# AlterPang/Multi_ORB_SLAM

Hardware: AMD Instinct MI355X
Metric: frames/sec (N-cam extract+match) (higher is better)
Workload: dtype u8; 1 GPU; configs[1]: one 2-cam 640x480 rig per GPU, 8-level pyramid, 1000 feat/cam; HIP FAST+rBRIEF extract + SearchByProjection + cross-camera Hamming top-2; cams_per_gpu=2, rig_cams=2, rigs=1, width=640, height=480, nfeatures=1000, nlevels=8, frame_unit=one rig timestep (2 cameras)

## Files before the change

multi_orb_slam_amd/csrc/resolve_dev.h:

```cpp
#pragma once
#include <hip/hip_runtime.h>
#include <cstddef>
#include <type_traits>
#include "../../include/orbm.h"
#include "orb_common.h"
#include "matcher_internal.h"

namespace morb {

static __host__ __device__ __forceinline__ int rotation_bin(float query_angle, float feature_angle) {
    float rot = query_angle - feature_angle;
    if (rot < 0.0) rot += 360.0f;
    int bin = (int)roundf(rot * (1.0f / ORBM_HISTO_LENGTH));
    if (bin == ORBM_HISTO_LENGTH) bin = 0;
    return (bin >= 0 && bin < ORBM_HISTO_LENGTH) ? bin : -1;
}

static __host__ __device__ __forceinline__ void three_maxima(const int* histo, int L, int* ind) {
    int m1 = 0, m2 = 0, m3 = 0, i1 = -1, i2 = -1, i3 = -1;
    for (int i = 0; i < L; i++) {
        const int s = histo[i];
        if (s > m1) { m3 = m2; i3 = i2; m2 = m1; i2 = i1; m1 = s; i1 = i; }
        else if (s > m2) { m3 = m2; i3 = i2; m2 = s; i2 = i; }
        else if (s > m3) { m3 = s; i3 = i; }
// ... 6 lines not shown
static __device__ __forceinline__ void three_maxima_wave(int sv, int lane, int keep[3]) {
    int rank = 0;
#pragma unroll
    for (int j = 0; j < ORBM_HISTO_LENGTH; ++j) {
        const int sj = __builtin_amdgcn_readlane(sv, j);
        rank += (sj > sv || (sj == sv && j < lane)) ? 1 : 0;
    }
    const bool in = lane < ORBM_HISTO_LENGTH && sv > 0;
    const unsigned long long r1 = __ballot(in && rank == 0), r2 = __ballot(in && rank == 1), r3 = __ballot(in && rank == 2);
    int i1 = r1 ? __ffsll((long long)r1) - 1 : -1, i2 = r2 ? __ffsll((long long)r2) - 1 : -1, i3 = r3 ? __ffsll((long long)r3) - 1 : -1;
    const int m1 = i1 >= 0 ? __builtin_amdgcn_readlane(sv, i1) : 0, m2 = i2 >= 0 ? __builtin_amdgcn_readlane(sv, i2) : 0,
              m3 = i3 >= 0 ? __builtin_amdgcn_readlane(sv, i3) : 0;
    if ((float)m2 < 0.1f * (float)m1) { i2 = -1; i3 = -1; }
    else if ((float)m3 < 0.1f * (float)m1) { i3 = -1; }
    keep[0] = i1; keep[1] = i2; keep[2] = i3;
}

static __device__ __forceinline__ void hist_add_wave(int* s_hist, bool in_range, int bin, int lane) {
    unsigned long long todo = __ballot(in_range);
    for (int rounds = 0; todo && rounds < 3; ++rounds) {
        const int b0 = __builtin_amdgcn_readlane(bin, __ffsll((long long)todo) - 1);
        const unsigned long long same = __ballot(in_range && bin == b0);
        if (in_range && bin == b0 && lane == __ffsll((long long)same) - 1) atomicAdd(&s_hist[b0], __popcll(same));
        todo &= ~same;
    }
    if (in_range && ((todo >> lane) & 1)) atomicAdd(&s_hist[bin], 1);
}

struct Rescan { int k1, g1, k2; };
template <bool SECOND, typename Hidden>
static __device__ __forceinline__ Rescan rescan_wave(int q, int full, int nq, const int* __restrict__ cand_idx,
                                                     const uint16_t* __restrict__ cand_dist, const uint8_t* __restrict__ occupied,
                                                     int lane, Hidden hidden) {
    int k1 = 0x7fffffff, k2 = 0x7fffffff, g1 = -1;
    for (int k0 = 0; k0 < full; k0 += 64) {
        const int k = k0 + lane;
        int key = 0x7fffffff, g = -1;
        if (k < full) {
            g = cand_idx[k * nq + q];
            const int d = cand_dist[k * nq + q];
            bool avail = !(occupied && occupied[g]);
            if (hidden(g, q)) avail = false;
            if (avail) key = (d << 16) | k;
        }
        const int m1 = (int)wave_min_u32((unsigned)key);
        int m2 = 0x7fffffff;
        if (SECOND) m2 = (int)wave_min_u32((unsigned)(key == m1 ? 0x7fffffff : key));
        if (m1 < k1) {
            k2 = min(k1, m2); k1 = m1;
            g1 = __builtin_amdgcn_readlane(g, __ffsll((long long)__ballot(key == m1)) - 1);
        }
        else k2 = min(k2, m1);
    }
    return {k1, g1, k2};
}

struct Advance { int nk, ne; };
template <int K>
static __device__ __forceinline__ void shortlist_claims(const int (&e)[K], int p, bool displaced, const int* claims, int (&ck)[K]) {
#pragma unroll
    for (int k = 1; k < K; ++k) {
        const bool want = displaced && k > p && e[k] != 0xffff;
        const int v = claims[want ? e[k] : 0];
        ck[k] = want ? v : -1;
    }
}
template <int K>
static __device__ __forceinline__ Advance shortlist_first_free(const int (&e)[K], const int (&ck)[K], int i) {
    int nk = K;
#pragma unroll
    for (int k = K - 1; k >= 1; --k) if (ck[k] >= i) nk = k;
    int ne = 0xffff;
#pragma unroll
    for (int k = 1; k < K; ++k) if (nk == k) ne = e[k];
    return {nk, ne};
}
template <int K>
static __device__ __forceinline__ Advance shortlist_advance(const int (&e)[K], int p, int i, const int* claims) {
    int ck[K];
    shortlist_claims(e, p, true, claims, ck);
    return shortlist_first_free(e, ck, i);
}

struct RescanCtx {
    int nq; const int* cand_idx; const uint16_t* cand_dist; const uint8_t* occupied; int th_high, f0;
};

template <int RQ, typename Choice, typename Len>
static __device__ inline bool mono_pass(int* claims, const int (&qi)[RQ], const int (&e)[RQ][RESOLVE_K], int (&c)[RQ], int (&p)[RQ],
                                                 const int (&fl)[RQ], Choice l_choice, const RescanCtx& R, Len list_len, int lane,
                                                 unsigned long long* chg) {
    constexpr int K = RESOLVE_K;
    constexpr bool MIRROR = !std::is_same<Choice, std::nullptr_t>::value;
    bool disp[RQ], need_rescan[RQ];
    int cl[RQ];
#pragma unroll
    for (int b = 0; b < RQ; ++b) cl[b] = claims[c[b] >= 0 ? c[b] : 0];
#pragma unroll
    for (int b = 0; b < RQ; ++b) { disp[b] = c[b] >= 0 && cl[b] < qi[b]; need_rescan[b] = false; }
    bool any = false;
#pragma unroll
    for (int b = 0; b < RQ; ++b) any |= disp[b];
    if (!__ballot(any)) return false;
    {
        int ck[RQ][K];
#pragma unroll
        for (int b = 0; b < RQ; ++b) {
            if (!__ballot(disp[b])) continue;
            shortlist_claims(e[b], p[b], disp[b], claims, ck[b]);
        }
#pragma unroll
        for (int b = 0; b < RQ; ++b) {
            if (!__ballot(disp[b])) continue;
            if (!disp[b]) continue;
            const int i = qi[b];
#ifdef MORB_PHASE_CLOCKS
            if (chg) atomicAdd(chg, 1ull);
#endif
            const Advance a = shortlist_first_free(e[b], ck[b], i);
            if (a.nk < K) {
                c[b] = a.ne; p[b] = a.nk;
                if constexpr (MIRROR) l_choice[i] = (unsigned short)a.ne;
                if (fl[b] & 1) atomicMin(&claims[a.ne], i);
            } else {
                c[b] = -1; p[b] = K;
                if constexpr (MIRROR) l_choice[i] = 0xffff;
                need_rescan[b] = (fl[b] & 2) != 0;
            }
        }
    }
#pragma unroll
    for (int b = 0; b < RQ; ++b) {
        unsigned long long todo = __ballot(need_rescan[b]);
#ifdef MORB_PHASE_CLOCKS
        if (todo && lane == 0 && chg) atomicAdd(chg + 16, (unsigned long long)__popcll(todo));
#endif
        while (todo) {
            const int src = __ffsll((long long)todo) - 1;
            todo &= todo - 1;
            const int q = __builtin_amdgcn_readlane(qi[b], src);
            const Rescan r = rescan_wave<false>(q, list_len(q), R.nq, R.cand_idx, R.cand_dist, R.occupied, lane,
                                                [&](int g, int q_) { return claims[g - R.f0] < q_; });
            if (lane == src && r.k1 != 0x7fffffff && (r.k1 >> 16) <= R.th_high) {
                const int g1 = r.g1 - R.f0;
                c[b] = g1;
                if constexpr (MIRROR) l_choice[q] = (unsigned short)g1;
                if (fl[b] & 1) atomicMin(&claims[g1], q);
            }
        }
    }
    return true;
}

static __device__ __forceinline__ void write_matches(int* __restrict__ words, const int* owner, int count, int tagb, int tid, int T) {
    for (int g = tid; g < count; g += T) words[g] = tagb ? (tagb | (owner[g] + 2)) : owner[g];
}
static __device__ __forceinline__ void write_no_match_tail(int* __restrict__ match_of_feature, int NT, int capacity, int tagb, int tid, int T) {
    if (tagb) for (int g = NT + tid; g < capacity; g += T) match_of_feature[g] = tagb | 1;
}

template <typename T>
static __device__ __forceinline__ T* lds_at(int* base, size_t byte_offset) {
    return reinterpret_cast<T*>(reinterpret_cast<unsigned char*>(base) + byte_offset);
}

struct JacobiLds {
    size_t n, nq;
    __host__ __device__ JacobiLds(int n_, int nq_) : n((size_t)n_), nq((size_t)nq_) {}
    __host__ __device__ size_t claim2() const { return 4 * n; }
    __host__ __device__ size_t cnt() const { return 8 * n; }
    __host__ __device__ size_t tables_bytes() const { return cnt() + (nq + 1) / 2 * 4; }
    __host__ __device__ size_t choice() const { return tables_bytes(); }
    __host__ __device__ size_t gd() const { return choice() + 4 * nq; }
    __host__ __device__ size_t ang() const { return gd() + 4 * RESOLVE_K * nq; }
    __host__ __device__ size_t fang() const { return ang() + 4 * nq; }
    __host__ __device__ size_t fl() const { return fang() + 4 * n; }
    __host__ __device__ size_t bytes(bool ldsq) const { return ldsq ? fl() + nq + 16 : tables_bytes(); }
};

struct MonoLds {
    size_t n, nq, nq2;
    bool with_ang;
    __host__ __device__ MonoLds(int n_, int nq_, bool ang_) : n((size_t)n_), nq((size_t)nq_), nq2(((size_t)nq_ + 1) & ~(size_t)1), with_ang(ang_) {}
    __host__ __device__ size_t owner() const { return 4 * n; }
    __host__ __device__ size_t cnt() const { return 8 * n; }
    __host__ __device__ size_t choice() const { return cnt() + 2 * nq2; }
    __host__ __device__ size_t gd() const { return choice() + 2 * nq2; }
    __host__ __device__ size_t fl() const { return gd() + 2 * RESOLVE_K * nq2; }
    __host__ __device__ size_t ang() const { return fl() + ((nq + 3) & ~(size_t)3); }
    __host__ __device__ size_t fang() const { return ang() + 4 * nq; }
    __host__ __device__ size_t wl() const { return with_ang ? fang() + 4 * n : ang(); }
    __host__ __device__ size_t bytes() const { return wl() + 2 * nq2 + 16; }
};

struct CamsLds {
    size_t nf_cap, q_cap;
    __host__ __device__ CamsLds(int nf_cap_, int q_cap_) : nf_cap((size_t)nf_cap_), q_cap((size_t)q_cap_) {}
    __host__ __device__ size_t owner() const { return 4 * nf_cap; }
    __host__ __device__ size_t queries() const { return 8 * nf_cap; }
    __host__ __device__ size_t bytes() const { return queries() + 2 * q_cap; }
};

}
```

multi_orb_slam_amd/csrc/search.hip:

```cpp
#include <algorithm>
#include <cmath>
#include <cstdlib>
#include <type_traits>
#include <vector>

#include "../../include/orbm.h"
#include "../../include/orb_debug.h"
#include "orb_common.h"
#include "frame_sink.h"
#include "matcher_internal.h"
#include "hamming_dev.h"
#include "project_dev.h"
#include "resolve_dev.h"

using namespace morb;

namespace {
__global__ __launch_bounds__(256) void k_project(ProjectArgs A) {
    MORB_LATENCY_KERNEL_WIDE();
    const int qi = __builtin_amdgcn_readfirstlane(blockIdx.x * 4 + (threadIdx.x >> 6));
    if (qi >= A.nq) return;
    project_wave(A, qi, threadIdx.x & 63);
}

// ... 189 lines not shown
                        else {
                            if (found == 0) { best = dk[k]; bidx = gk[k]; }
                            else { best2 = dk[k]; g2 = gk[k]; }
                            if (++found >= NEED) walking = false;
                        }
                    }
                };
#pragma unroll
                for (int k = 0; k < K0; ++k) fetch(k);
#pragma unroll
                for (int k = 0; k < K0; ++k) ck[k] = gk[k] >= 0 ? rd[gk[k]] : 0x7fffffff;
#pragma unroll
                for (int k = 0; k < K0; ++k) walk(k);
                if (__ballot(walking)) {
#pragma unroll
                    for (int k = K0; k < RESOLVE_K; ++k) fetch(k);
#pragma unroll
                    for (int k = K0; k < RESOLVE_K; ++k) ck[k] = gk[k] >= 0 ? rd[gk[k]] : 0x7fffffff;
#pragma unroll
                    for (int k = K0; k < RESOLVE_K; ++k) walk(k);
                }
                if (POINTS) { if (bidx >= 0) lvl = F.octave[bidx]; if (g2 >= 0) lvl2 = F.octave[g2]; }
                need_rescan = found < NEED && (fl & 2) && taken > 0;
                if (!need_rescan && best <= th_high && bidx >= 0) {
                    nc = bidx;
                    if (POINTS && lvl == lvl2 && (float)best > nnratio * (float)best2) nc = -1;
                }
            }
            unsigned long long todo = __ballot(need_rescan);
#ifdef MORB_PHASE_CLOCKS
            if (todo && lane == 0 && it < 15) atomicAdd(&s_nres, __popcll(todo));
#endif
            while (todo) {
                const int src = __ffsll((long long)todo) - 1;
                todo &= todo - 1;
                const int qi = __builtin_amdgcn_readlane(i, src);
                const Rescan r = rescan_wave<POINTS>(qi, l_cnt[qi], nq, cand_idx, cand_dist, occupied, lane,
                                                     [&](int g, int q) { return (unsigned)(rd[g] - tag) < (unsigned)q; });
                int best = 256, best2 = 256, lvl = -1, lvl2 = -1, bidx = -1;
                if (r.k1 != 0x7fffffff) {
                    best = r.k1 >> 16; bidx = r.g1;
                    if (POINTS) lvl = F.octave[bidx];
                }
                if (POINTS && r.k2 != 0x7fffffff) { best2 = r.k2 >> 16; lvl2 = F.octave[cand_idx[(r.k2 & 0xffff) * nq + qi]]; }
                int rnc = -1;
                if (best <= th_high && bidx >= 0) {
                    rnc = bidx;
                    if (POINTS && lvl == lvl2 && (float)best > nnratio * (float)best2) rnc = -1;
                }
                if (lane == src) nc = rnc;
            }
            if (valid) {
#ifdef MORB_PHASE_CLOCKS
                if (nc != old && it < 15) atomicAdd((unsigned long long*)&g_ph_chg[it], 1ull);
#endif
                if (nc != old) { ch = 1; if (LDSQ) l_choice[i] = nc; else choice[i] = nc; }
                if constexpr (B < RQ) chr[B] = nc;
                if (nc >= 0 && (fl & 1)) atomicMin(&wr[nc], tag_next | i);
            }
        };
        batch(0, std::integral_constant<int, 0>{});
        if (T < nq) batch(T, std::integral_constant<int, 1>{});
        if constexpr (RQ > 2) {
            if (2 * T < nq) batch(2 * T, std::integral_constant<int, 2>{});
            if (3 * T < nq) batch(3 * T, std::integral_constant<int, 3>{});
        }
        for (int base = RQ * T; base < nq; base += T) batch(base, std::integral_constant<int, RQ>{});
#ifdef MORB_PHASE_CLOCKS
        __syncthreads();
        if (tid == 0 && it < 15) g_ph_res[40 + it] = (unsigned long long)s_nres;
#endif
        if (it == 0) MORB_PHASE(g_ph_res, 20); else if (it == 5) MORB_PHASE(g_ph_res, 24);
        if (it == 0) MORB_PHASE(g_ph_res, 22); else if (it == 5) MORB_PHASE(g_ph_res, 26);
        changed = __syncthreads_or(ch);
        MORB_PHASE(g_ph_res, min(3 + it, 50));
    }
    if (changed) {
        if (tid == 0) { status[1] = tagb | 0; status[2] = tagb | it; status[3] = tagb | maxcount; status[0] = tagb | 1; }
        return;
    }
    for (int g = tid; g < NT; g += T) s_claim[g] = -1;
    if (tid < ORBM_HISTO_LENGTH) s_hist[tid] = 0;
    if (tid == 0) s_red = 0;
    __syncthreads();
    MORB_PHASE(g_ph_res, 52);
    auto bin_of = [&](int i, int c) { return LDSQ ? rotation_bin(l_ang[i], l_fang[c]) : rotation_bin(__int_as_float(qmeta[i].y), f_angle[c]); };
    int acc = 0;
    for (int i = tid; i < nq; i += T) {
        const int c = LDSQ ? l_choice[i] : choice[i];
        if (c < 0) continue;
        ++acc;
        atomicMax(&s_claim[c], i);
        if (!POINTS && check_ori) {
            const int bin = bin_of(i, c);
            if (LDSQ) l_fl[i] = (unsigned char)((l_fl[i] & 3) | ((bin + 1) << 2));
            hist_add_wave(s_hist, bin >= 0, bin, lane);
        }
    }
    acc = __builtin_amdgcn_readlane(wave_incl_scan(acc), 63);
    if (lane == 0) atomicAdd(&s_red, acc);
    __syncthreads();
    MORB_PHASE(g_ph_res, 53);
    if (!POINTS && check_ori) {
        if (tid < 64) {
            int keep[3];
            three_maxima_wave(tid < ORBM_HISTO_LENGTH ? s_hist[tid] : 0, lane, keep);
            if (tid == 0) { s_keep[0] = keep[0]; s_keep[1] = keep[1]; s_keep[2] = keep[2]; }
        }
        __syncthreads();
        MORB_PHASE(g_ph_res, 54);
        int rej = 0;
        for (int i = tid; i < nq; i += T) {
            const int c = LDSQ ? l_choice[i] : choice[i];
            if (c < 0) continue;
            const int bin = LDSQ ? (int)(l_fl[i] >> 2) - 1 : bin_of(i, c);
            if (bin >= 0 && bin != s_keep[0] && bin != s_keep[1] && bin != s_keep[2]) {
                s_claim[c] = -2;
                ++rej;
            }
        }
        rej = __builtin_amdgcn_readlane(wave_incl_scan(rej), 63);
        if (lane == 0) atomicSub(&s_red, rej);
        __syncthreads();
    }
    MORB_PHASE(g_ph_res, 60);
    write_matches(match_of_feature, s_claim, NT, tagb, tid, T);
    write_no_match_tail(match_of_feature, NT, F.n_total, tagb, tid, T);
    if (tid == 0) { status[1] = tagb | s_red; status[2] = tagb | it; status[3] = tagb | maxcount; status[0] = tagb | 0; }
    MORB_PHASE(g_ph_res, 61);
#ifdef MORB_PHASE_CLOCKS
    if (tid == 0) g_ph_res[62] = (unsigned long long)it;
#endif
}

template <int RQ, bool ANG>
__global__ __launch_bounds__(1024) void k_resolve_mono(FrameDev F, const int2* __restrict__ qmeta, int nq, int cap,
                                                       const int* __restrict__ cand_idx, const uint16_t* __restrict__ cand_dist,
                                                       const int* __restrict__ cand_count, const uint8_t* __restrict__ occupied,
                                                       const float* __restrict__ f_angle, int th_high, int check_ori, int max_it,
                                                       const int* __restrict__ topk, int* __restrict__ match_of_feature,
                                                       int* __restrict__ status, int tagb, MergeJob MJ, int worklist) {
    MORB_LATENCY_KERNEL();
    if (blockIdx.x > 0) { merge_carrier_block(MJ, 1); return; }
    extern __shared__ __attribute__((aligned(16))) int s_claim[];
    __shared__ int s_hist[ORBM_HISTO_LENGTH];
    __shared__ int s_merge_ok;
    __shared__ int s_keep[3];
    __shared__ int s_red;
    __shared__ int s_flag[3];
    const int tid = threadIdx.x, T = blockDim.x;
    const int lane = tid & 63;
    MORB_PHASE(g_ph_res, 0);
#ifdef MORB_PHASE_CLOCKS
    if (tid == 0) { g_ph_res[1] = 0; g_ph_res[58] = clock64(); }
#endif
    if (tid < 3) s_flag[tid] = 0;
    const int NT = F.n_total_dev ? *F.n_total_dev : F.n_total;
    const int* tk_g = topk + RESOLVE_K * nq;
    const MonoLds L(F.n_total, nq, ANG);
    const int nq2 = (int)L.nq2;
    int* s_owner = lds_at<int>(s_claim, L.owner());
    unsigned short* l_cnt = lds_at<unsigned short>(s_claim, L.cnt());
    unsigned short* l_choice = lds_at<unsigned short>(s_claim, L.choice());
    unsigned short* l_gd = lds_at<unsigned short>(s_claim, L.gd());
    unsigned char* l_fl = lds_at<unsigned char>(s_claim, L.fl());
    float* l_ang = lds_at<float>(s_claim, L.ang());
    float* l_fang = lds_at<float>(s_claim, L.fang());
    unsigned short* l_wl = lds_at<unsigned short>(s_claim, L.wl());
    __shared__ int s_wl_n[2];
    if (tid == 0) s_red = 0;
    if (tid < ORBM_HISTO_LENGTH) s_hist[tid] = 0;
    for (int g = tid; g < F.n_total; g += T) {
        s_claim[g] = 0x7fffffff; s_owner[g] = -1;
        if (ANG && check_ori) l_fang[g] = f_angle[g];
    }
    __syncthreads();
    constexpr int K = RESOLVE_K;
    int sl[RQ][K], cur[RQ], pos[RQ], flr[RQ];
    int mx = 0;
    auto setup = [&](const int i, int (&e)[K], int& c, int& fl) {
        const int cnt_i = cand_count[i];
        mx = max(mx, cnt_i);
        l_cnt[i] = (unsigned short)min(cnt_i, 65535);
        const int2 qm = qmeta[i];
        fl = (qm.x & 1) | (topk[(2 * K) * nq + i] > K ? 2 : 0);
        l_fl[i] = (unsigned char)fl;
        if (ANG) l_ang[i] = __int_as_float(qm.y);
#pragma unroll
        for (int k = 0; k < K; ++k) {
            e[k] = tk_g[k * nq + i] & 0xffff;
            l_gd[k * nq2 + i] = (unsigned short)e[k];
        }
        const bool has = e[0] != 0xffff;
        c = has ? e[0] : -1;
        l_choice[i] = (unsigned short)(has ? e[0] : 0xffff);
        if (has && (fl & 1)) atomicMin(&s_claim[e[0]], i);
    };
#pragma unroll
    for (int b = 0; b < RQ; ++b) {
        const int i = b * T + tid;
        cur[b] = -1; pos[b] = 0; flr[b] = 0;
#pragma unroll
        for (int k = 0; k < K; ++k) sl[b][k] = 0xffff;
        if (i < nq) setup(i, sl[b], cur[b], flr[b]);
    }
    for (int i = RQ * T + tid; i < nq; i += T) { int e[K], c, fl; setup(i, e, c, fl); }
    mx = (int)(0x7fffffffu - wave_min_u32(0x7fffffffu - (unsigned)mx));
    if (lane == 0) atomicMax(&s_red, mx);
    __syncthreads();
    const int maxcount = s_red;
    if (maxcount > cap) {
        (void)merge_wait(MJ, &s_merge_ok);
        if (tid == 0) { status[1] = tagb | 0; status[2] = tagb | 0; status[3] = tagb | maxcount; status[0] = tagb | 2; }
        return;
    }
    MORB_PHASE(g_ph_res, 2);
    const RescanCtx RC{nq, cand_idx, cand_dist, occupied, th_high, 0};
    int it = 1, changed = 1;
    auto pass = [&](const int (&qi)[RQ], const int (&e)[RQ][K], int (&c)[RQ], int (&p)[RQ], const int (&fl)[RQ]) -> bool {
        [[clang::always_inline]] return mono_pass<RQ>(s_claim, qi, e, c, p, fl, l_choice, RC, [&](int q) { return (int)l_cnt[q]; }, lane, MORB_CHG_SLOT(it));
    };
    if (worklist) {
        if (tid < 2) s_wl_n[tid] = 0;
        __syncthreads();
        for (; it < max_it; ++it) {
            int* cnt = &s_wl_n[it & 1];
            for (int i0 = 0; i0 < nq; i0 += RQ * T) {
                int cc[RQ], cl[RQ];
#pragma unroll
                for (int b = 0; b < RQ; ++b) { const int i = i0 + b * T + tid; cc[b] = i < nq ? (int)l_choice[i] : 0xffff; }
#pragma unroll
                for (int b = 0; b < RQ; ++b) cl[b] = s_claim[cc[b] != 0xffff ? cc[b] : 0];
#pragma unroll
                for (int b = 0; b < RQ; ++b) {
                    const int i = i0 + b * T + tid;
                    const bool disp = cc[b] != 0xffff && cl[b] < i;
                    const unsigned long long m = __ballot(disp);
                    if (m) {
                        int base = 0;
                        if (lane == __ffsll((long long)m) - 1) base = atomicAdd(cnt, __popcll(m));
                        base = __builtin_amdgcn_readlane(base, __ffsll((long long)m) - 1);
                        if (disp) l_wl[base + __popcll(m & ((1ull << lane) - 1ull))] = (unsigned short)i;
                    }
                }
            }
            if (tid == 0) s_wl_n[(it + 1) & 1] = 0;
            __syncthreads();
            const int nwl = *cnt;
#ifdef MORB_PHASE_CLOCKS
            if (tid == 0 && it < 15) atomicAdd((unsigned long long*)&g_ph_chg[it], (unsigned long long)nwl);
#endif
            if (nwl == 0) { changed = 0; break; }
            for (int j0 = 0; j0 < nwl; j0 += T) {
                const int j = j0 + tid;
                const int i = j < nwl ? (int)l_wl[j] : -1;
                bool need_rescan = false;
                int fl = 0;
                if (i >= 0) {
                    fl = l_fl[i];
                    const int c = l_choice[i];
                    int e[K], p = K;
#pragma unroll
                    for (int k = 0; k < K; ++k) e[k] = l_gd[k * nq2 + i];
#pragma unroll
                    for (int k = K - 1; k >= 0; --k) if (e[k] == c) p = k;
                    const Advance a = shortlist_advance(e, p, i, s_claim);
                    l_choice[i] = (unsigned short)a.ne;
                    if (a.nk < K) { if (fl & 1) atomicMin(&s_claim[a.ne], i); }
                    else need_rescan = (fl & 2) != 0;
                }
                unsigned long long todo = __ballot(need_rescan);
                while (todo) {
                    const int src = __ffsll((long long)todo) - 1;
                    todo &= todo - 1;
                    const int q = __builtin_amdgcn_readlane(i, src);
                    const Rescan r = rescan_wave<false>(q, l_cnt[q], nq, cand_idx, cand_dist, occupied, lane,
                                                        [&](int g, int q_) { return s_claim[g] < q_; });
                    if (lane == src && r.k1 != 0x7fffffff && (r.k1 >> 16) <= th_high) {
                        l_choice[q] = (unsigned short)r.g1;
                        if (fl & 1) atomicMin(&s_claim[r.g1], q);
                    }
                }
            }
            __syncthreads();
            MORB_PHASE(g_ph_res, min(2 + it, 50));
        }
    } else {
    int qi01[RQ];
#pragma unroll
    for (int b = 0; b < RQ; ++b) qi01[b] = b * T + tid;
    for (; it < max_it && changed; ++it) {
        if (tid == 0) s_flag[(it + 1) % 3] = 0;
        bool ch = false;
        for (int guard = 0; guard < 4096; ++guard) {
            bool w = pass(qi01, sl, cur, pos, flr);
            for (int base = RQ * T; base < nq; base += RQ * T) {
                int qx[RQ], e[RQ][K], c[RQ], p[RQ], fl[RQ];
#pragma unroll
                for (int b = 0; b < RQ; ++b) {
                    const int i = base + b * T + tid;
                    qx[b] = i; c[b] = -1; p[b] = K; fl[b] = 0;
#pragma unroll
                    for (int k = 0; k < K; ++k) e[b][k] = 0xffff;
                    if (i < nq) {
                        fl[b] = l_fl[i];
                        const int g = l_choice[i] == 0xffff ? -1 : (int)l_choice[i];
#pragma unroll
                        for (int k = 0; k < K; ++k) e[b][k] = l_gd[k * nq2 + i];
                        c[b] = g;
#pragma unroll
                        for (int k = K - 1; k >= 0; --k) if (g >= 0 && e[b][k] == g) p[b] = k;
                    }
                }
                w |= pass(qx, e, c, p, fl);
            }
            if (!w) {
#ifdef MORB_PHASE_CLOCKS
                if (lane == 0 && it < 15) atomicMax((unsigned long long*)&g_ph_chg[32 + it], (unsigned long long)guard);
                if (lane == 0 && it == 1 && blockIdx.x == 0) g_ph_chg[48 + (tid >> 6)] = ((unsigned long long)guard << 32) | (unsigned long long)(wall_clock64() - g_ph_res[0]);
#endif
                break;
            }
            ch = true;
        }
        if (ch && lane == 0) s_flag[it % 3] = 1;
        __syncthreads();
        changed = s_flag[it % 3];
        MORB_PHASE(g_ph_res, min(2 + it, 50));
    }
    }
    if (changed) {
        (void)merge_wait(MJ, &s_merge_ok);
        if (tid == 0) { status[1] = tagb | 0; status[2] = tagb | it; status[3] = tagb | maxcount; status[0] = tagb | 1; }
        return;
    }
    if (tid == 0) s_red = 0;
    __syncthreads();
    MORB_PHASE(g_ph_res, 52);
    int acc = 0;
    for (int i = tid; i < nq; i += T) {
        const int c = l_choice[i] == 0xffff ? -1 : (int)l_choice[i];
        if (c < 0) continue;
        ++acc;
        atomicMax(&s_owner[c], i);
        if (check_ori) {
            const int bin = ANG ? rotation_bin(l_ang[i], l_fang[c]) : rotation_bin(__int_as_float(qmeta[i].y), f_angle[c]);
            l_fl[i] = (unsigned char)((l_fl[i] & 3) | ((bin + 1) << 2));
            hist_add_wave(s_hist, bin >= 0, bin, lane);
        }
    }
    acc = __builtin_amdgcn_readlane(wave_incl_scan(acc), 63);
    if (lane == 0) atomicAdd(&s_red, acc);
    __syncthreads();
    MORB_PHASE(g_ph_res, 53);
    if (check_ori) {
        if (tid < 64) {
            int keep[3];
            three_maxima_wave(tid < ORBM_HISTO_LENGTH ? s_hist[tid] : 0, lane, keep);
            if (tid == 0) { s_keep[0] = keep[0]; s_keep[1] = keep[1]; s_keep[2] = keep[2]; }
        }
        __syncthreads();
        MORB_PHASE(g_ph_res, 54);
        int rej = 0;
        for (int i = tid; i < nq; i += T) {
            const int c = l_choice[i] == 0xffff ? -1 : (int)l_choice[i];
            if (c < 0) continue;
            const int bin = (int)(l_fl[i] >> 2) - 1;
            if (bin >= 0 && bin != s_keep[0] && bin != s_keep[1] && bin != s_keep[2]) {
                s_owner[c] = -2;
                ++rej;
            }
        }
        rej = __builtin_amdgcn_readlane(wave_incl_scan(rej), 63);
        if (lane == 0) atomicSub(&s_red, rej);
        __syncthreads();
    }
    MORB_PHASE(g_ph_res, 60);
    const bool merged = merge_wait(MJ, &s_merge_ok);
    write_matches(match_of_feature, s_owner, NT, tagb, tid, T);
    write_no_match_tail(match_of_feature, NT, F.n_total, tagb, tid, T);
    if (tid == 0) { status[1] = tagb | s_red; status[2] = tagb | it; status[3] = tagb | maxcount; status[0] = tagb | (merged ? 0 : 3); }
    MORB_PHASE(g_ph_res, 61);
#ifdef MORB_PHASE_CLOCKS
    if (tid == 0) { g_ph_res[62] = (unsigned long long)it; g_ph_res[59] = clock64(); }
#endif
}

constexpr int RS_MAX_SWEEPS = 24;
constexpr int RS_STATE_INTS = 80;

__global__ __launch_bounds__(256) void k_rs_init(int n_cap, int nq, int* __restrict__ tab0, int* __restrict__ tab1,
                                                 int* __restrict__ owner, int* __restrict__ choice,
                                                 const int* __restrict__ cand_count, int* __restrict__ state, int n_sweeps) {
    const int i = blockIdx.x * 256 + threadIdx.x;
    if (i == 0) state[5] = n_sweeps;
    if (i < n_cap) { tab0[i] = 0x7fffffff; tab1[i] = 0x7fffffff; owner[i] = -1; }
    int mx = 0;
    if (i < nq) { choice[i] = -1; mx = cand_count[i]; }
#pragma unroll
    for (int o = 32; o > 0; o >>= 1) mx = max(mx, __shfl_xor(mx, o));
    if ((threadIdx.x & 63) == 0 && mx > 0) atomicMax(&state[0], mx);
}

template <bool POINTS>
__global__ __launch_bounds__(256) void k_rs_sweep(FrameDev F, const orbm_query* __restrict__ q, int nq, int cap, int it,
                                                  const int* __restrict__ cand_idx, const uint16_t* __restrict__ cand_dist,
                                                  const int* __restrict__ cand_count, const uint8_t* __restrict__ occupied,
                                                  int th_high, float nnratio, int* __restrict__ choice,
                                                  const int* __restrict__ topk, const int* __restrict__ rd,
                                                  int* __restrict__ wr, int* __restrict__ state) {
    if (state[0] > cap) return;
    if (it > 0 && state[8 + it - 1] == 0) return;
    const int i = blockIdx.x * 256 + threadIdx.x;
    constexpr int NEED = POINTS ? 2 : 1;
    const int tag = (0x7ffe - it) << 16, tag_next = (0x7ffd - it) << 16;
    int ch = 0;
    if (i < nq) {
        const int* tk_key = topk;
        const int* tk_g = topk + RESOLVE_K * nq;
        int sg[RESOLVE_K], sd[RESOLVE_K];
#pragma unroll
        for (int k = 0; k < RESOLVE_K; ++k) { sg[k] = tk_g[k * nq + i]; sd[k] = tk_key[k * nq + i] >> 16; }
        const bool longer = topk[(2 * RESOLVE_K) * nq + i] > RESOLVE_K;
        const int old = choice[i], bl = q[i].blocks;
        int best = 256, best2 = 256, lvl = -1, lvl2 = -1, bidx = -1;
        int found = 0, taken = 0;
#pragma unroll
        for (int k = 0; k < RESOLVE_K; ++k) {
            if (found >= NEED) break;
            const int g = sg[k];
            if (g < 0) break;
            const int cl = rd[g];
            if ((cl >> 16) == (tag >> 16) && (cl & 0xffff) < i) { ++taken; continue; }
            if (found == 0) { best = sd[k]; bidx = g; if (POINTS) lvl = F.octave[g]; }
            else { best2 = sd[k]; lvl2 = F.octave[g]; }
            ++found;
        }
        if (found < NEED && longer && taken > 0) {
// ... 475 lines not shown
        const int32_t* ci = m->h_i0.p + (size_t)i * cap;
        const uint16_t* cd = m->h_u16.p + (size_t)i * cap;
        int best = 256, best2 = 256, lvl = -1, lvl2 = -1, bidx = -1;
        for (int k = 0; k < cnt; k++) {
            const int g = ci[k];
            const int owner = match_of_feature[g];
            if (owner >= 0 ? q[owner].blocks != 0 : (occupied && occupied[g])) continue;
            const int d = cd[k];
            if (points) {
                if (d < best) { best2 = best; best = d; lvl2 = lvl; lvl = cur->octave[g]; bidx = g; }
                else if (d < best2) { lvl2 = cur->octave[g]; best2 = d; }
            } else if (d < best) { best = d; bidx = g; }
        }
        if (best <= th_high && bidx >= 0) {
            if (points && lvl == lvl2 && (float)best > nnratio * (float)best2) continue;
            match_of_feature[bidx] = i;
            nm++;
            if (!points && check_orientation) {
                const int bin = rotation_bin(q[i].angle, cur->angle[bidx]);
                if (bin >= 0) rot[bin].push_back(bidx);
            }
        }
    }
    if (!points && check_orientation) {
        int sizes[ORBM_HISTO_LENGTH], ind[3];
        for (int b = 0; b < ORBM_HISTO_LENGTH; b++) sizes[b] = (int)rot[b].size();
        orbm_three_maxima(sizes, ORBM_HISTO_LENGTH, ind);
        for (int b = 0; b < ORBM_HISTO_LENGTH; b++)
            if (b != ind[0] && b != ind[1] && b != ind[2])
                for (int g : rot[b]) { match_of_feature[g] = -2; nm--; }
    }
    *nmatches = nm;
    return ORB_OK;
}

int morb::search_enqueue(orbm_matcher* m, SearchJob& J, bool queries_already_on_device) {
    const int n = J.cur->n_total;
    J.device_path = false; J.pollable = false; J.multi = false;
    J.form = ORBM_FORM_NONE;
    if (J.nq == 0 || n == 0) return ORB_OK;
    J.form = ORBM_FORM_HOST;
    constexpr size_t LDS_LIMIT = 150 * 1024;
    const JacobiLds jacobi(n, J.nq);
    const bool multi = jacobi.bytes(false) > LDS_LIMIT;
    if (m->host_resolve || J.nq > RESOLVE_MAX_Q) return ORB_OK;
    if (multi) { int rcg = m->d_gclaim.reserve((size_t)2 * n + RS_STATE_INTS); if (rcg) return rcg; }
    int rc;
    if ((rc = m->d_choice.reserve(J.nq)) || (rc = m->d_claim.reserve((size_t)(2 * RESOLVE_K + 1) * J.nq)) || (rc = m->d_match.reserve(n)) ||
        (rc = m->d_status.reserve(4)) || (rc = m->h_match.reserve((size_t)n + 4)) || (rc = m->d_occ.reserve(std::max(n, 16))))
        return rc;
    if (J.occupied && !J.occ_dev) MORB_HIP(hipMemcpyAsync(m->d_occ.p, J.occupied, (size_t)n, hipMemcpyHostToDevice, m->stream));
    const uint8_t* d_occ = J.occ_dev ? J.occ_dev : (J.occupied ? m->d_occ.p : nullptr);
    const orbm_frame* cur = J.cur;
    const int nq = J.nq, cap = J.cap, th_high = J.th_high;
    const float nnratio = J.nnratio;
    if ((rc = m->d_qmeta.reserve(nq))) return rc;
    const orbm_query* q_in_place = (J.q_dev && !multi) ? J.q_dev : nullptr;
    if (J.q_dev && multi && !J.msrc) {
        if ((rc = m->d_queries.reserve((size_t)nq * sizeof(orbm_query)))) return rc;
        MORB_HIP(hipMemcpyAsync(m->d_queries.p, J.q_dev, (size_t)nq * sizeof(orbm_query), hipMemcpyDefault, m->stream));
    }
    MergeJob MJ{nullptr, nullptr, nullptr, 0, 0, nullptr, nullptr, nullptr, nullptr};
    if ((rc = run_project(m, cur, J.q, nq, cap, 1, 1, !queries_already_on_device && !J.q_dev && !J.msrc, false, 1, d_occ,
                          m->d_claim.p, J.points ? 256 : th_high, nullptr, q_in_place, m->d_qmeta.p, J.win2_dev, J.side, J.msrc, multi,
                          (J.side && !multi && !J.points) ? &MJ : nullptr)))
        return rc;
    J.side = nullptr;
    J.seq = 0;
    if (J.want_tags) { m->resolve_seq = m->resolve_seq % 2047 + 1; J.seq = m->resolve_seq; }
    static const int cam_env = [] { const char* e = getenv("MORB_RS_PER_CAMERA"); return e ? atoi(e) : 1; }();
    const int cams_min_q = cam_env > 1 ? cam_env : 0x7fffffff;
    int nf_cap = 0, q_cam_max = J.q_cam_max;
    QRanges QR; QR.n = 0;
    const bool starts_ok = cur->camera_major && (int)cur->cam_start.size() == cur->n_cams + 1 && cur->cam_start[cur->n_cams] == n;
    const bool cams_want = cam_env && !J.points && !J.win2_dev && starts_ok && (multi || (cur->n_cams >= 2 && nq >= cams_min_q));
    if (cams_want) {
        for (int c = 0; c < cur->n_cams; ++c) nf_cap = std::max(nf_cap, cur->cam_start[c + 1] - cur->cam_start[c]);
        if (!q_cam_max && !J.msrc && J.q) {
            std::vector<int>& per = m->rs_cam_count;
            per.assign((size_t)cur->n_cams, 0);
            bool sorted = cur->n_cams <= 64;
            int last = 0;
            for (int i = 0; i < nq; ++i) {
                const int c = J.q[i].cam;
                if (c >= 0 && c < cur->n_cams) q_cam_max = std::max(q_cam_max, ++per[c]);
                if (c < last || c >= cur->n_cams) sorted = false; else last = c;
            }
            if (!q_cam_max) q_cam_max = 1;
            if (sorted) { QR.n = cur->n_cams; int b = 0; for (int c = 0; c < cur->n_cams; ++c) { QR.start[c] = b; b += per[c]; } QR.start[cur->n_cams] = b; }
        } else if (J.q_cam_start && cur->n_cams <= 64 && J.q_cam_start[cur->n_cams] == nq) {
            QR.n = cur->n_cams;
            for (int c = 0; c <= cur->n_cams; ++c) QR.start[c] = J.q_cam_start[c];
        }
    }
    const size_t lds_cam = CamsLds(nf_cap, RSC_RQ * 1024).bytes();
    const bool cams_fit = cams_want && nf_cap > 0 && q_cam_max > 0 && q_cam_max <= RSC_RQ * 1024 && nq < 65536 && lds_cam <= LDS_LIMIT;
    auto launch_cams = [&](MergeJob MJc, int merge_blocks) -> int {
        int rcl;
        if (!m->d_rsync.p) {
            if ((rcl = m->d_rsync.reserve(RS_STATE_INTS))) return rcl;
            MORB_HIP(hipMemsetAsync(m->d_rsync.p, 0, RS_STATE_INTS * sizeof(int), m->stream));
        }
        hipLaunchKernelGGL(k_resolve_cams, dim3(cur->n_cams + merge_blocks), dim3(1024), lds_cam, m->stream, cur->dev(), (const int*)cur->b->d_cam_start.p,
                           (const int2*)m->d_qmeta.p, nq, cap, nf_cap, (const int*)m->d_i0.p, (const uint16_t*)m->d_u16.p,
                           (const int*)m->d_i1.p, d_occ, (const float*)cur->b->d_ang.p, th_high, J.check_ori, 4096,
                           (const int*)m->d_claim.p, m->d_rsync.p, m->h_match.dp + 4, m->h_match.dp, J.seq << 20, cur->n_cams, MJc, QR);
        MORB_HIP(hipGetLastError());
        return ORB_OK;
    };
    if (multi) {
        int* tab0 = m->d_gclaim.p; int* tab1 = tab0 + n; int* state = tab1 + n;
        if (!cams_fit) MORB_HIP(hipMemsetAsync(state, 0, RS_STATE_INTS * sizeof(int), m->stream));
        const int nb_all = (std::max(n, nq) + 255) / 256, nb_q = (nq + 255) / 256, nb_f = (n + 255) / 256;
        if (cams_fit) {
            if ((rc = launch_cams(MergeJob{nullptr, nullptr, nullptr, 0, 0, nullptr, nullptr, nullptr, nullptr}, 0))) return rc;
            J.device_path = true; J.form = ORBM_FORM_CAMS;
            J.pollable = J.seq != 0;
            return ORB_OK;
        }
        J.seq = 0;
        const int n_sweeps = std::min(RS_MAX_SWEEPS, std::max(12, m->rs_sweeps_hint));
        hipLaunchKernelGGL(k_rs_init, dim3(nb_all), dim3(256), 0, m->stream, n, nq, tab0, tab1, m->d_match.p, m->d_choice.p,
                           (const int*)m->d_i1.p, state, n_sweeps);
        J.multi = true;
        const auto sweep = J.points ? k_rs_sweep<true> : k_rs_sweep<false>;
        for (int it = 0; it < n_sweeps; ++it) {
            const int* rd = (it & 1) ? tab1 : tab0;
            int* wr = (it & 1) ? tab0 : tab1;
            hipLaunchKernelGGL(sweep, dim3(nb_q), dim3(256), 0, m->stream, cur->dev(), (const orbm_query*)m->d_queries.p, nq,
                               cap, it, (const int*)m->d_i0.p, (const uint16_t*)m->d_u16.p, (const int*)m->d_i1.p, d_occ, th_high,
                               nnratio, m->d_choice.p, (const int*)m->d_claim.p, rd, wr, state);
        }
        const int ori = J.points ? 0 : J.check_ori;
        hipLaunchKernelGGL(k_rs_owner, dim3(nb_q), dim3(256), 0, m->stream, (const orbm_query*)m->d_queries.p, nq, cap,
                           (const int*)m->d_choice.p, (const float*)cur->b->d_ang.p, ori, m->d_match.p, state);
        if (ori)
            hipLaunchKernelGGL(k_rs_reject, dim3(nb_q), dim3(256), 0, m->stream, (const orbm_query*)m->d_queries.p, nq, cap,
                               (const int*)m->d_choice.p, (const float*)cur->b->d_ang.p, m->d_match.p, state);
        hipLaunchKernelGGL(k_rs_write, dim3(nb_f), dim3(256), 0, m->stream, n, cur->dev().n_total_dev, cap, (const int*)m->d_match.p,
                           (const int*)state, m->h_match.dp + 4, m->h_match.dp);
        MORB_HIP(hipGetLastError());
        J.device_path = true; J.form = ORBM_FORM_SWEEPS;
        return ORB_OK;
    }
    const bool ldsq = jacobi.bytes(true) <= LDS_LIMIT && n < 65535;
    const size_t lds_use = jacobi.bytes(ldsq);
#define MORB_RESOLVE_LAUNCH(PT, LQ)                                                                                      \
    hipLaunchKernelGGL((k_resolve<PT, LQ>), dim3(1), dim3(1024), lds_use, m->stream, cur->dev(), (const int2*)m->d_qmeta.p, \
                       nq, cap, (const int*)m->d_i0.p, (const uint16_t*)m->d_u16.p, (const int*)m->d_i1.p, d_occ,            \
                       (const float*)cur->b->d_ang.p, th_high, nnratio, J.points ? 0 : J.check_ori, 256, m->d_choice.p,      \
                       (const int*)m->d_claim.p, m->h_match.dp + 4, m->h_match.dp, J.seq << 20)
    static const int mono_mode = [] { const char* e = getenv("MORB_RESOLVE_MONO"); return e ? atoi(e) : 2; }();
    const bool mono_env = mono_mode != 0;
    const int mono_worklist = mono_mode == 2 && nq > 2048 ? 1 : 0;
    const bool will_mono = !J.points && mono_env && n < 65535 && MonoLds(n, nq, false).bytes() <= LDS_LIMIT;
    if (MJ.S > 1 && !will_mono && !cams_fit) { if ((rc = launch_merge(m->stream, MJ))) return rc; MJ.S = 0; }
    int merge_blocks = 0;
    auto carry_merge = [&]() -> int {
        merge_blocks = MJ.S > 1 ? (MJ.nq + 1023) / 1024 : 0;
        if (!merge_blocks) return ORB_OK;
        int rcm = m->d_mergecnt.reserve(4);
        if (rcm) return rcm;
        if (!m->merge_ready) { MORB_HIP(hipMemsetAsync(m->d_mergecnt.p, 0, 16, m->stream)); m->merge_ready = true; m->merge_target = 0; }
        m->merge_target += (unsigned)merge_blocks;
        MJ.done = reinterpret_cast<unsigned*>(m->d_mergecnt.p); MJ.target = m->merge_target;
        return ORB_OK;
    };
    if (cams_fit) {
        if ((rc = carry_merge()) || (rc = launch_cams(MJ, merge_blocks))) return rc;
        MJ.S = 0;
        J.form = ORBM_FORM_CAMS;
    } else if (will_mono) {
        const bool ang = MonoLds(n, nq, true).bytes() <= LDS_LIMIT;
        const size_t ml = MonoLds(n, nq, ang).bytes();
#define MORB_MONO_LAUNCH(RQ_, ANG_)                                                                                                       \
        hipLaunchKernelGGL((k_resolve_mono<RQ_, ANG_>), dim3(1 + merge_blocks), dim3(1024), ml, m->stream, cur->dev(), (const int2*)m->d_qmeta.p, nq, cap, \
                           (const int*)m->d_i0.p, (const uint16_t*)m->d_u16.p, (const int*)m->d_i1.p, d_occ,                                \
                           (const float*)cur->b->d_ang.p, th_high, J.check_ori, 4096, (const int*)m->d_claim.p, m->h_match.dp + 4,          \
                           m->h_match.dp, J.seq << 20, MJ, mono_worklist)
        if ((rc = carry_merge())) return rc;
        if (nq <= 2048) { if (ang) MORB_MONO_LAUNCH(2, true); else MORB_MONO_LAUNCH(2, false); }
        else { if (ang) MORB_MONO_LAUNCH(4, true); else MORB_MONO_LAUNCH(4, false); }
        MJ.S = 0;
        J.form = nq <= 2048 ? (ang ? ORBM_FORM_MONO2_ANG : ORBM_FORM_MONO2) : (mono_worklist ? ORBM_FORM_MONO4_WORKLIST : ORBM_FORM_MONO4_WAVES);
#undef MORB_MONO_LAUNCH
    } else if (ldsq) { if (J.points) MORB_RESOLVE_LAUNCH(true, true); else MORB_RESOLVE_LAUNCH(false, true); J.form = ORBM_FORM_JACOBI_LDSQ; }
    else { if (J.points) MORB_RESOLVE_LAUNCH(true, false); else MORB_RESOLVE_LAUNCH(false, false); J.form = ORBM_FORM_JACOBI; }
#undef MORB_RESOLVE_LAUNCH
    MORB_HIP(hipGetLastError());
    J.device_path = true;
    J.pollable = J.seq != 0;
    return ORB_OK;
}

int morb::search_finish(orbm_matcher* m, SearchJob& J, int32_t* match_of_feature, int* nmatches) {
    const int n = J.cur->n_total;
    *nmatches = 0;
    m->last_form[0] = J.device_path ? J.form : (J.nq == 0 || n == 0 ? ORBM_FORM_NONE : ORBM_FORM_HOST); m->last_form[1] = 0;
    if (J.nq == 0 || n == 0) { for (int g = 0; g < n; g++) match_of_feature[g] = -1; return ORB_OK; }
    if (!J.device_path) {
        m->last_status[0] = -1; m->last_status[1] = 0; m->last_status[2] = 0; m->last_status[3] = 0;
    }
    auto need_q = [&] { if (J.q_fill) { J.q_fill(J.q_fill_ctx); J.q_fill = nullptr; } };
    if (!J.device_path) {
        need_q();
        return host_resolve(m, J.cur, J.q, J.nq, J.occupied, J.points, J.nnratio, J.th_high, J.check_ori, 64, match_of_feature, nmatches, J.win2_dev);
    }
    bool synced = false;
    auto word = [&](int idx, int bias) -> int {
        volatile int32_t* p = m->h_match.p + idx;
        if (!J.seq) return *p;
        for (int spin = 0;; ++spin) {
            const int w = *p;
            if ((w >> 20) == J.seq) return (w & 0xfffff) - bias;
            if (spin > 100000 && !synced) { (void)hipStreamSynchronize(m->stream); synced = true; spin = 0; }
            else if (spin > 100000) return -3;
            __builtin_ia32_pause();
        }
    };
    for (;;) {
        const int status = word(0, 0);
        m->last_status[0] = status;
        for (int k = 1; k < 4; ++k) m->last_status[k] = word(k, 0);
        if (status == -3) { morb::set_error("resolve results never arrived"); return ORB_E_HIP; }
        if (J.multi) m->rs_sweeps_hint = status == 0 ? m->last_status[2] + 4 : RS_MAX_SWEEPS;
        if (status != 0 && !synced) { MORB_HIP(hipStreamSynchronize(m->stream)); synced = true; }
        if (status == 0 || status == 3) { m->last_status[0] = 0; break; }
        if (status == 2) {
            J.cap = (m->last_status[3] + 63) & ~63;
            int rc = search_enqueue(m, J, true);
            if (rc) return rc;
            m->last_form[0] = J.form; m->last_form[1]++;
            MORB_HIP(hipStreamSynchronize(m->stream));
            synced = true;
            continue;
        }
        need_q();
        m->last_form[0] = ORBM_FORM_HOST;
        return host_resolve(m, J.cur, J.q, J.nq, J.occupied, J.points, J.nnratio, J.th_high, J.check_ori, J.cap, match_of_feature, nmatches, J.win2_dev);
    }
    if (J.seq) {
        for (int g = 0; g < n; ++g) {
            const int v = word(4 + g, 2);
            if (v == -3) { morb::set_error("resolve results never arrived"); return ORB_E_HIP; }
            match_of_feature[g] = v;
        }
    } else if (match_of_feature != m->h_match.p + 4) memcpy(match_of_feature, m->h_match.p + 4, (size_t)n * 4);
    *nmatches = m->last_status[1];
    return ORB_OK;
}

static int search_common(orbm_matcher* m, const orbm_frame* cur, const orbm_query* q, int nq, const uint8_t* occupied,
                         bool points, float nnratio, int th_high, int check_orientation, int32_t* match_of_feature,
                         int* nmatches, const orbm_window* second = nullptr) {
    SearchJob J{cur, q, nq, occupied, points, nnratio, th_high, check_orientation, 64, false};
    int rc;
    if (second && nq > 0) {
        if ((rc = m->d_win2.reserve(nq))) return rc;
        MORB_HIP(hipMemcpyAsync(m->d_win2.p, second, (size_t)nq * sizeof(orbm_window), hipMemcpyHostToDevice, m->stream));
        MORB_HIP(hipStreamSynchronize(m->stream));
        J.win2_dev = m->d_win2.p;
    }
    if (nq > 0 && cur->n_total > 0 && !m->host_resolve && nq <= RESOLVE_MAX_Q) {
        const size_t qbytes = ((size_t)nq * sizeof(orbm_query) + 255) & ~(size_t)255, obytes = occupied ? (size_t)cur->n_total : 0;
        if ((rc = m->stage_q.reserve(qbytes + obytes + 16))) return rc;
        memcpy(m->stage_q.p, q, (size_t)nq * sizeof(orbm_query));
        if (occupied) memcpy(m->stage_q.p + qbytes, occupied, obytes);
        m->stage_q.publish();
        J.q_dev = reinterpret_cast<const orbm_query*>(m->stage_q.dp);
        J.occ_dev = occupied ? m->stage_q.dp + qbytes : nullptr;
    }
    rc = search_enqueue(m, J);
    if (rc) return rc;
    if (J.device_path) MORB_HIP(hipStreamSynchronize(m->stream));
    return search_finish(m, J, match_of_feature, nmatches);
}

int orbm_search_by_projection(orbm_matcher* m, const orbm_frame* cur, const orbm_query* q, int nq,
                              const uint8_t* occupied, int th_high, int check_orientation, int32_t* match_of_feature,
                              int* nmatches) {
    MORB_ARG(m && cur && nq >= 0 && nmatches && (cur->n_total == 0 || match_of_feature) && (nq == 0 || q));
    MORB_HIP(hipSetDevice(m->device));
    return search_common(m, cur, q, nq, occupied, false, 0.f, th_high, check_orientation, match_of_feature, nmatches);
}

int orbm_search_by_projection_windows(orbm_matcher* m, const orbm_frame* cur, const orbm_query* q, const orbm_window* second, int nq,
                                      const uint8_t* occupied, int th_high, int check_orientation, int32_t* match_of_feature,
                                      int* nmatches) {
    MORB_ARG(m && cur && nq >= 0 && nmatches && (cur->n_total == 0 || match_of_feature) && (nq == 0 || (q && second)));
    MORB_HIP(hipSetDevice(m->device));
    return search_common(m, cur, q, nq, occupied, false, 0.f, th_high, check_orientation, match_of_feature, nmatches, second);
}

int orbm_search_by_projection_points(orbm_matcher* m, const orbm_frame* cur, const orbm_query* q, int nq,
                                     const uint8_t* occupied, float nnratio, int th_high, int32_t* match_of_feature,
                                     int* nmatches) {
    MORB_ARG(m && cur && nq >= 0 && nmatches && (cur->n_total == 0 || match_of_feature) && (nq == 0 || q));
    MORB_HIP(hipSetDevice(m->device));
    std::vector<orbm_query> q0(q, q + nq);
    for (auto& Q : q0) Q.cam = 0;
    return search_common(m, cur, q0.data(), nq, occupied, true, nnratio, th_high, 0, match_of_feature, nmatches);
}
```

Before: 24690 frames/s.

## Make mono resolve worklist wave-local to drop block barriers per iteration

Replaces the block-wide worklist iteration in the mono resolve kernel with per-wave worklists. Each wave owns a slice of queries and propagates displaced claims directly: atomicMin reports the loser, which becomes the next item, so the per-iteration __syncthreads and global rescan of all queries are removed. A final block-level sweep fixes non-claiming queries, and the worklist path is now enabled for all query counts rather than only nq > 2048. This risks load imbalance between waves and relies on workgroup fences for cross-wave visibility of choices and claims.

```diff
diff --git a/multi_orb_slam_amd/csrc/resolve_dev.h b/multi_orb_slam_amd/csrc/resolve_dev.h
--- a/multi_orb_slam_amd/csrc/resolve_dev.h
+++ b/multi_orb_slam_amd/csrc/resolve_dev.h
@@ -182,6 +182,58 @@
     return true;
 }
 
+static __device__ __forceinline__ int claim_and_report(int* claims, int g, int i) {
+    const int old = atomicMin(&claims[g], i);
+    return old < i ? i : (old > i && old != 0x7fffffff ? old : -1);
+}
+
+template <typename Len>
+static __device__ __forceinline__ int displaced_step(int* claims, int i, unsigned short* l_choice, const unsigned short* l_gd, int nq2,
+                                                     const unsigned char* l_fl, const RescanCtx& R, Len list_len, int lane,
+                                                     unsigned long long* chg) {
+    constexpr int K = RESOLVE_K;
+    bool need_rescan = false;
+    int fl = 0, next = -1;
+    if (i >= 0) {
+        fl = l_fl[i];
+        const int c = l_choice[i];
+        int e[K], p = K;
+#pragma unroll
+        for (int k = 0; k < K; ++k) e[k] = l_gd[k * nq2 + i];
+#pragma unroll
+        for (int k = K - 1; k >= 0; --k) if (e[k] == c) p = k;
+        const Advance a = shortlist_advance(e, p, i, claims);
+        l_choice[i] = (unsigned short)a.ne;
+        __builtin_amdgcn_fence(__ATOMIC_RELEASE, "workgroup");
+        if (a.nk < K) { if (fl & 1) next = claim_and_report(claims, a.ne, i); }
+        else need_rescan = (fl & 2) != 0;
+    }
+    unsigned long long todo = __ballot(need_rescan);
+#ifdef MORB_PHASE_CLOCKS
+    if (todo && lane == 0 && chg) atomicAdd(chg + 16, (unsigned long long)__popcll(todo));
+#endif
+    while (todo) {
+        const int src = __ffsll((long long)todo) - 1;
+        todo &= todo - 1;
+        const int q = __builtin_amdgcn_readlane(i, src);
+        const Rescan r = rescan_wave<false>(q, list_len(q), R.nq, R.cand_idx, R.cand_dist, R.occupied, lane,
+                                            [&](int g, int q_) { return claims[g - R.f0] < q_; });
+        if (lane == src && r.k1 != 0x7fffffff && (r.k1 >> 16) <= R.th_high) {
+            const int g1 = r.g1 - R.f0;
+            l_choice[q] = (unsigned short)g1;
+            __builtin_amdgcn_fence(__ATOMIC_RELEASE, "workgroup");
+            if (fl & 1) next = claim_and_report(claims, g1, q);
+        }
+    }
+    return next;
+}
+
+static __device__ __forceinline__ int worklist_append(unsigned short* list, int base, int v, int lane) {
+    const unsigned long long m = __ballot(v >= 0);
+    if (v >= 0) list[base + __popcll(m & ((1ull << lane) - 1ull))] = (unsigned short)v;
+    return __popcll(m);
+}
+
 static __device__ __forceinline__ void write_matches(int* __restrict__ words, const int* owner, int count, int tagb, int tid, int T) {
     for (int g = tid; g < count; g += T) words[g] = tagb ? (tagb | (owner[g] + 2)) : owner[g];
 }
diff --git a/multi_orb_slam_amd/csrc/search.hip b/multi_orb_slam_amd/csrc/search.hip
--- a/multi_orb_slam_amd/csrc/search.hip
+++ b/multi_orb_slam_amd/csrc/search.hip
@@ -365,7 +365,7 @@
     const int lane = tid & 63;
     MORB_PHASE(g_ph_res, 0);
 #ifdef MORB_PHASE_CLOCKS
-    if (tid == 0) { g_ph_res[1] = 0; g_ph_res[58] = clock64(); }
+    if (tid == 0) { g_ph_res[1] = 0; g_ph_res[63] = (unsigned long long)worklist; g_ph_res[58] = clock64(); }
 #endif
     if (tid < 3) s_flag[tid] = 0;
     const int NT = F.n_total_dev ? *F.n_total_dev : F.n_total;
@@ -380,7 +380,6 @@
     float* l_ang = lds_at<float>(s_claim, L.ang());
     float* l_fang = lds_at<float>(s_claim, L.fang());
     unsigned short* l_wl = lds_at<unsigned short>(s_claim, L.wl());
-    __shared__ int s_wl_n[2];
     if (tid == 0) s_red = 0;
     if (tid < ORBM_HISTO_LENGTH) s_hist[tid] = 0;
     for (int g = tid; g < F.n_total; g += T) {
@@ -434,69 +433,45 @@
         [[clang::always_inline]] return mono_pass<RQ>(s_claim, qi, e, c, p, fl, l_choice, RC, [&](int q) { return (int)l_cnt[q]; }, lane, MORB_CHG_SLOT(it));
     };
     if (worklist) {
-        if (tid < 2) s_wl_n[tid] = 0;
+        const int slice = (nq + T - 1) / T * 64;
+        const int q0 = min(nq, (tid >> 6) * slice), q1 = min(nq, q0 + slice);
+        unsigned short* const list = l_wl + q0;
+        auto len_of = [&](int q) { return (int)l_cnt[q]; };
+        int n = 0;
+        for (int i0 = q0; i0 < q1; i0 += 64) {
+            const int i = i0 + lane;
+            const int c = i < q1 ? (int)l_choice[i] : 0xffff;
+            const int cl = s_claim[c != 0xffff ? c : 0];
+            n += worklist_append(list, n, c != 0xffff && cl < i ? i : -1, lane);
+        }
+        for (; n > 0 && it < max_it; ++it) {
+#ifdef MORB_PHASE_CLOCKS
+            if (lane == 0 && it < 15) atomicAdd((unsigned long long*)&g_ph_chg[it], (unsigned long long)n);
+#endif
+            __builtin_amdgcn_fence(__ATOMIC_SEQ_CST, "wavefront");
+            __builtin_amdgcn_wave_barrier();
+            int m = 0;
+            for (int j0 = 0; j0 < n; j0 += 64) {
+                const int i = j0 + lane < n ? (int)list[j0 + lane] : -1;
+                m += worklist_append(list, m, displaced_step(s_claim, i, l_choice, l_gd, nq2, l_fl, RC, len_of, lane, MORB_CHG_SLOT(it)), lane);
+            }
+            n = m;
+            MORB_PHASE(g_ph_res, min(2 + it, 50));
+        }
+#ifdef MORB_PHASE_CLOCKS
+        if (tid == 0) g_ph_res[57] = (unsigned long long)it;
+#endif
+        if (lane == 0) { atomicMax(&s_flag[1], it); if (n > 0) s_flag[0] = 1; }
         __syncthreads();
-        for (; it < max_it; ++it) {
-            int* cnt = &s_wl_n[it & 1];
-            for (int i0 = 0; i0 < nq; i0 += RQ * T) {
-                int cc[RQ], cl[RQ];
-#pragma unroll
-                for (int b = 0; b < RQ; ++b) { const int i = i0 + b * T + tid; cc[b] = i < nq ? (int)l_choice[i] : 0xffff; }
-#pragma unroll
-                for (int b = 0; b < RQ; ++b) cl[b] = s_claim[cc[b] != 0xffff ? cc[b] : 0];
-#pragma unroll
-                for (int b = 0; b < RQ; ++b) {
-                    const int i = i0 + b * T + tid;
-                    const bool disp = cc[b] != 0xffff && cl[b] < i;
-                    const unsigned long long m = __ballot(disp);
-                    if (m) {
-                        int base = 0;
-                        if (lane == __ffsll((long long)m) - 1) base = atomicAdd(cnt, __popcll(m));
-                        base = __builtin_amdgcn_readlane(base, __ffsll((long long)m) - 1);
-                        if (disp) l_wl[base + __popcll(m & ((1ull << lane) - 1ull))] = (unsigned short)i;
-                    }
-                }
-            }
-            if (tid == 0) s_wl_n[(it + 1) & 1] = 0;
-            __syncthreads();
-            const int nwl = *cnt;
-#ifdef MORB_PHASE_CLOCKS
-            if (tid == 0 && it < 15) atomicAdd((unsigned long long*)&g_ph_chg[it], (unsigned long long)nwl);
-#endif
-            if (nwl == 0) { changed = 0; break; }
-            for (int j0 = 0; j0 < nwl; j0 += T) {
-                const int j = j0 + tid;
-                const int i = j < nwl ? (int)l_wl[j] : -1;
-                bool need_rescan = false;
-                int fl = 0;
-                if (i >= 0) {
-                    fl = l_fl[i];
-                    const int c = l_choice[i];
-                    int e[K], p = K;
-#pragma unroll
-                    for (int k = 0; k < K; ++k) e[k] = l_gd[k * nq2 + i];
-#pragma unroll
-                    for (int k = K - 1; k >= 0; --k) if (e[k] == c) p = k;
-                    const Advance a = shortlist_advance(e, p, i, s_claim);
-                    l_choice[i] = (unsigned short)a.ne;
-                    if (a.nk < K) { if (fl & 1) atomicMin(&s_claim[a.ne], i); }
-                    else need_rescan = (fl & 2) != 0;
-                }
-                unsigned long long todo = __ballot(need_rescan);
-                while (todo) {
-                    const int src = __ffsll((long long)todo) - 1;
-                    todo &= todo - 1;
-                    const int q = __builtin_amdgcn_readlane(i, src);
-                    const Rescan r = rescan_wave<false>(q, l_cnt[q], nq, cand_idx, cand_dist, occupied, lane,
-                                                        [&](int g, int q_) { return s_claim[g] < q_; });
-                    if (lane == src && r.k1 != 0x7fffffff && (r.k1 >> 16) <= th_high) {
-                        l_choice[q] = (unsigned short)r.g1;
-                        if (fl & 1) atomicMin(&s_claim[r.g1], q);
-                    }
-                }
-            }
-            __syncthreads();
-            MORB_PHASE(g_ph_res, min(2 + it, 50));
+        changed = s_flag[0]; it = s_flag[1];
+        MORB_PHASE(g_ph_res, 51);
+        if (!changed) {
+            for (int i0 = 0; i0 < nq; i0 += T) {
+                const int i = i0 + tid;
+                bool d = false;
+                if (i < nq && !(l_fl[i] & 1)) { const int c = l_choice[i]; d = c != 0xffff && s_claim[c] < i; }
+                if (__ballot(d)) (void)displaced_step(s_claim, d ? i : -1, l_choice, l_gd, nq2, l_fl, RC, len_of, lane, nullptr);
+            }
         }
     } else {
     int qi01[RQ];
@@ -1278,7 +1253,7 @@
                        (const int*)m->d_claim.p, m->h_match.dp + 4, m->h_match.dp, J.seq << 20)
     static const int mono_mode = [] { const char* e = getenv("MORB_RESOLVE_MONO"); return e ? atoi(e) : 2; }();
     const bool mono_env = mono_mode != 0;
-    const int mono_worklist = mono_mode == 2 && nq > 2048 ? 1 : 0;
+    const int mono_worklist = mono_mode == 2 ? 1 : 0;
     const bool will_mono = !J.points && mono_env && n < 65535 && MonoLds(n, nq, false).bytes() <= LDS_LIMIT;
     if (MJ.S > 1 && !will_mono && !cams_fit) { if ((rc = launch_merge(m->stream, MJ))) return rc; MJ.S = 0; }
     int merge_blocks = 0;
```

Result: faster. 25920 frames/s (median of 6 runs) (+5.0%).
